# gleb-kov/wordpiece

Hardware: NVIDIA B200
Metric: GB/s text tokenized (higher is better)
Workload: dtype u8

## Files before the change

wordpiece_b200/csrc/wp_encode.cu:

```cuda
#include <cuda_runtime.h>
#include <stddef.h>
#include <stdint.h>

#include "wp_encode.h"
#include "wp_table.h"

#ifdef WP_DEBUG_BOUNDS
#include <cstdio>
#define WP_CHECK(cond)                                                                                              \
  do {                                                                                                              \
    if (!(cond)) {                                                                                                  \
      printf("WP_CHECK failed: %s (wp_encode.cu:%d, block %d, thread %d)\n", #cond, __LINE__, static_cast<int>(blockIdx.x), \
             static_cast<int>(threadIdx.x));                                                                        \
      __trap();                                                                                                     \
    }                                                                                                               \
  } while (0)
#else
#define WP_CHECK(cond) \
  do {                 \
  } while (0)
#endif

namespace wp {

constexpr int TILE = 4096;
constexpr int CHUNK = 32;
constexpr int THREADS = 160;
constexpr int HALO = 256;
constexpr int LOOKAHEAD = 32;
constexpr int LEFT = 16;
constexpr int WINDOW = TILE + HALO;
constexpr int NCHUNK = WINDOW / CHUNK;
constexpr int OWNED_CHUNKS = TILE / CHUNK;
constexpr int RAW_BYTES = LEFT + WINDOW + LOOKAHEAD;
constexpr int WARPS = THREADS / 32;
constexpr int MAX_TILE_SLOW = TILE / 2 + 8;
constexpr int PREFETCH_TILES = 2 * 6 * 148;
constexpr uint32_t FULL = 0xFFFFFFFFu;
constexpr uint32_t POS_MASK = 0x3FFFu;
constexpr uint32_t SLOW_LONG = 0x8000u;

#ifndef WP_K2_BLOCKS
#define WP_K2_BLOCKS 5
#endif
#ifndef WP_K2_THREADS
#define WP_K2_THREADS 256
#endif
#ifndef WP_K1_PER_TURN
#define WP_K1_PER_TURN 2
#endif
#ifndef WP_K3_BLOCKS
#define WP_K3_BLOCKS 4
#endif
#ifndef WP_K1_SEG_CAP
#define WP_K1_SEG_CAP 3072
#endif
constexpr int MATCH_THREADS = WP_K2_THREADS;
constexpr int SCATTER_THREADS = 256;
constexpr int SCATTER_ITEMS = 8;
constexpr int SCATTER_SEGS = SCATTER_THREADS * SCATTER_ITEMS;
constexpr int SCATTER_STAGE = 6144;
#ifndef WP_SCATTER_BIG
#define WP_SCATTER_BIG 8
#endif
constexpr int SCATTER_BIG = WP_SCATTER_BIG;

static_assert(RAW_BYTES % 16 == 0, "raw buffer is loaded in 16-byte units");
static_assert(WORD_KEY_BYTES + 4 <= LOOKAHEAD, "key window reads stay inside the loaded bytes");
static_assert(LONG_SEGMENT_BYTES <= HALO, "a segment that starts in the tile and is not LONG ends inside the window");
static_assert(NCHUNK + 1 <= THREADS, "one thread per chunk in the classification and compaction passes");
static_assert(WINDOW <= static_cast<int>(POS_MASK), "positions must fit the packed list entries");
static_assert(TILE <= 4096, "segment ordinals must fit 12 bits of the tile slow list");
static_assert(NCHUNK < 256, "chunk indices are kept in bytes (hi_list)");

template <int SEG_CAP>
struct __align__(16) TileSmemT {
  uint8_t raw[RAW_BYTES];
  uint16_t seg_s[SEG_CAP];
  uint16_t seg_e[SEG_CAP + HALO + 64];
  uint16_t slow[MAX_TILE_SLOW];
  uint32_t dyn_hits;
  uint32_t n_eligible;
  uint32_t any_single;
  uint32_t m_lead[NCHUNK + 1];
  uint32_t m_space[NCHUNK + 1];
  uint32_t m_punct[NCHUNK + 1];
  uint32_t m_han[NCHUNK + 1];
  uint32_t m_cover[NCHUNK + 1];
  uint32_t m_kept[NCHUNK + 1];
  uint32_t kept_scan[NCHUNK + 2];
  uint8_t spill[NCHUNK + 1];
  uint8_t hi_list[NCHUNK + 8];
  uint32_t n_hi;
  uint32_t tile_ticket;
  uint4 key_mask[WORD_KEY_BYTES + 1];
  uint32_t warp_sums[WARPS];
  uint32_t prev_class;
  uint32_t left_spill;
  uint32_t n_segs;
  uint32_t n_ends;
  uint32_t n_slow;
  uint32_t slow_base;
  uint32_t arena_base;
  unsigned long long seg_base;
};
// ... 277 lines not shown
      sp |= (cls == CLS_SPACE ? 1u : 0u) << j;
      pu |= (cls == CLS_PUNCT ? 1u : 0u) << j;
      ha |= (cls == CLS_HAN ? 1u : 0u) << j;
    }
  } else {
    lead = 0;
    cover = 0;
    spill = 0;
    sp = 0;
    pu = 0;
    for (int j = 0; j < CHUNK; j++) {
      const uint32_t b0 = cb[j];
      if (is_cont_byte(b0)) continue;
      uint32_t cp = 0;
      const uint32_t len = b0 < 0x80u ? (cp = b0, 1u) : utf8_decode(b0, cb[j + 1], cb[j + 2], cb[j + 3], 4u, &cp);
      if (len == 0) continue;
      lead |= 1u << j;
      cover |= ((1u << len) - 1u) << j;
      if (j + static_cast<int>(len) > CHUNK) spill = j + len - CHUNK;
      const uint32_t cls = cp_class(cp);
      sp |= (cls == CLS_SPACE ? 1u : 0u) << j;
      pu |= (cls == CLS_PUNCT ? 1u : 0u) << j;
      ha |= (cls == CLS_HAN ? 1u : 0u) << j;
    }
  }
  const uint32_t in = limit_mask(c, limit);
  sm.m_lead[c] = lead & in;
  sm.m_space[c] = sp & in;
  sm.m_punct[c] = pu & in;
  sm.m_han[c] = ha & in;
  sm.m_cover[c] = cover;
  sm.spill[c] = static_cast<uint8_t>(spill);
}

template <class TileSmem>
__device__ __noinline__ void classify_window(TileSmem &sm, const uint8_t *buf, int limit) {
  const int tid = threadIdx.x;
  const int lane = tid & 31;
  const bool high = tid < NCHUNK && classify_ascii(sm, buf, tid, limit);
  const uint32_t hm = __ballot_sync(FULL, high);
  if (hm) {
    uint32_t at = 0;
    const int leader = __ffs(hm) - 1;
    if (lane == leader) at = smem_add(&sm.n_hi, static_cast<uint32_t>(__popc(hm)));
    at = __shfl_sync(FULL, at, leader);
    WP_CHECK(!high || at + __popc(hm & ((1u << lane) - 1u)) < NCHUNK + 8);
    if (high) sm.hi_list[at + __popc(hm & ((1u << lane) - 1u))] = static_cast<uint8_t>(tid);
  }
  __syncthreads();
  const uint32_t n_hi = sm.n_hi;
  for (uint32_t i = tid; i < n_hi; i += THREADS) classify_multibyte(sm, buf, sm.hi_list[i], limit);
}

template <int NWARPS>
__device__ __forceinline__ uint32_t block_exclusive_scan(uint32_t *warp_sums, uint32_t v, uint32_t *total) {
  const int lane = threadIdx.x & 31, warp = threadIdx.x >> 5;
  uint32_t incl = v;
#pragma unroll
  for (int o = 1; o < 32; o <<= 1) {
    const uint32_t y = __shfl_up_sync(FULL, incl, o);
    if (lane >= o) incl += y;
  }
  __syncthreads();
  if (lane == 31) warp_sums[warp] = incl;
  __syncthreads();
  uint32_t wbase = 0, tot = 0;
#pragma unroll
  for (int wi = 0; wi < NWARPS; wi++) {
    const uint32_t ws = warp_sums[wi];
    if (wi < warp) wbase += ws;
    tot += ws;
  }
  *total = tot;
  return wbase + incl - v;
}

__device__ __noinline__ unsigned long long tile_exclusive_scan(uint32_t *warp_sums, uint32_t v) {
  uint32_t total;
  const uint32_t at = block_exclusive_scan<WARPS>(warp_sums, v, &total);
  return (static_cast<unsigned long long>(total) << 32) | at;
}

__device__ __forceinline__ void lookback_publish(volatile unsigned long long *state, uint32_t index,
                                                 unsigned long long total) {
  state[index] = ((index == 0 ? 2ull : 1ull) << 62) | total;
}

constexpr uint32_t LOOKBACK_SPIN_LIMIT = 1u << 24;

__device__ __forceinline__ unsigned long long lookback_walk(volatile unsigned long long *state, uint32_t index,
                                                            unsigned long long total, int lane,
                                                            unsigned int *stalled = nullptr, unsigned int *void_call = nullptr) {
  constexpr unsigned long long VALUE_MASK = (1ull << 62) - 1;
  unsigned long long base = 0;
  if (index == 0) return 0;
  long long pred = static_cast<long long>(index) - 1 - lane;
  for (;;) {
    unsigned long long sv = 2ull << 62;
    if (pred >= 0) {
      uint32_t spins = 0;
      do {
        sv = state[pred];
        if (++spins > LOOKBACK_SPIN_LIMIT && stalled != nullptr) {
          *stalled = 1u;
          if (void_call != nullptr) *void_call = 1u;
          sv = 2ull << 62;
        }
      } while ((sv >> 62) == 0);
    }
    const uint32_t is_prefix = __ballot_sync(FULL, (sv >> 62) == 2);
    const int stop = is_prefix ? __ffs(is_prefix) - 1 : 31;
    unsigned long long v = lane <= stop ? (sv & VALUE_MASK) : 0ull;
#pragma unroll
    for (int o = 16; o > 0; o >>= 1) v += __shfl_xor_sync(FULL, v, o);
    base += v;
    if (is_prefix) break;
    pred -= 32;
  }
  if (lane == 0) state[index] = (2ull << 62) | (base + total);
  return base;
}

// ... 856 lines not shown
          sm.jump[k][i] = j == LONG_END ? static_cast<uint16_t>(LONG_END) : sm.jump[k - 1][j];
        }
        __syncthreads();
      }
#pragma unroll 1
      for (int k = LONG_LEVELS - 1; k >= 0; k--) {
        for (uint32_t i = tid; i < n; i += LONG_THREADS) {
          const uint32_t r = sm.rank[i];
          if (r == LONG_END) continue;
          const uint32_t j = sm.jump[k][i];
          WP_CHECK(j == LONG_END || (j < n && j > i && r + (1u << k) < LONG_BLOCK));
          if (j != LONG_END) sm.rank[j] = static_cast<uint16_t>(r + (1u << k));
        }
        __syncthreads();
      }
#pragma unroll 1
      for (uint32_t i = tid; i < n; i += LONG_THREADS) {
        const uint32_t r = sm.rank[i];
        if (r == LONG_END) continue;
        const uint32_t dl = sm.delta[i];
        if (dl == 0) {
          sm.failed = 1;
        } else {
          WP_CHECK(static_cast<unsigned long long>(sm.off) + n_out + r < P.arena_capacity && b0 + i - start >= n_out + r);
          out[n_out + r] = sm.id[i];
          if (sm.jump[0][i] == LONG_END) {
            sm.n_round = r + 1;
            sm.cur_next = b0 + i + dl;
          }
        }
      }
      __syncthreads();
      if (tid == 0) {
        sm.n_out = n_out + sm.n_round;
        sm.cur = sm.cur_next;
        if (sm.failed || sm.cur_next >= seg_end) sm.finished = 1;
      }
      __syncthreads();
    }
    if (tid == 0) {
      uint32_t cnt = sm.n_out;
      if (sm.failed) {
        cnt = sm.word_first + 1;
        P.arena[sm.off + sm.word_first] = static_cast<uint32_t>(V.unk_id);
      }
      if (P.call->overflow) cnt = 0;
      *reinterpret_cast<uint4 *>(&P.slow[si]) = make_uint4(cnt, sm.off, 0u, 0u);
      P.seg_result[ent.seg] = SEG_RESULT_SLOW | (min(cnt, SEG_SLOW_COUNT_MAX) << SEG_SLOW_INDEX_BITS) | si;
    }
  }
}


struct ScatterSmem {
  int32_t stage[SCATTER_STAGE];
  uint32_t desc_pos[SCATTER_SEGS];
  uint32_t desc_src[SCATTER_SEGS];
  uint32_t n_desc;
  uint32_t n_big;
  uint16_t big[SCATTER_STAGE / (SCATTER_BIG < 6144 ? SCATTER_BIG : 6144) + 2];
  uint32_t warp_sums[SCATTER_THREADS / 32];
  uint32_t block_index[2];
  unsigned long long base;
};

template <class Params>
__device__ __forceinline__ void scatter_fetch(const Params &P, uint32_t res, uint32_t cnt, int32_t *dst) {
  if (res & SEG_RESULT_SLOW) {
    const uint32_t si = res & SEG_SLOW_INDEX_MASK;
    if (si >= P.slow_capacity) return;
    const uint4 e = *reinterpret_cast<const uint4 *>(&P.slow[si]);
    if (e.x & SLOW_RESULT_INLINE) {
      dst[0] = static_cast<int32_t>(e.y);
      if (cnt > 1) dst[1] = static_cast<int32_t>(e.z);
      if (cnt > 2) dst[2] = static_cast<int32_t>(e.w);
    } else if (static_cast<unsigned long long>(e.y) + cnt <= P.arena_capacity) {
      const int32_t *src = reinterpret_cast<const int32_t *>(P.arena + e.y);
      for (uint32_t t = 0; t < cnt; t++) dst[t] = src[t];
    }
  } else {
    const WordSlot *slot = P.words + (res & SEG_WORD_SLOT_MASK);
    const uint4 e = *reinterpret_cast<const uint4 *>(&slot->meta);
    dst[0] = static_cast<int32_t>(e.y);
    if (cnt > 1) dst[1] = static_cast<int32_t>(e.z);
    if (cnt > 2) dst[2] = static_cast<int32_t>(e.w);
    for (uint32_t t = 3; t < cnt; t++) dst[t] = slot->ids[t];
  }
}

__device__ __forceinline__ void scatter_direct(const EncodeParams &P, unsigned long long first, unsigned long long n_segs,
                                            unsigned long long out0, uint32_t at, uint32_t *big_at, uint32_t *big_si,
                                            uint32_t *n_big) {
  unsigned long long o = out0 + at;
#pragma unroll 1
  for (int j = 0; j < SCATTER_ITEMS; j++) {
    if (first + j >= n_segs) break;
    const uint32_t res = P.seg_result[first + j];
    uint32_t cnt = 1u;
    if (res >= SEG_RESULT_WORD) {
      cnt = (res >> SEG_SLOW_INDEX_BITS) & ((res & SEG_RESULT_SLOW) ? SEG_SLOW_COUNT_MAX : 0xFu);
      if (cnt == SEG_SLOW_COUNT_MAX && (res & SEG_RESULT_SLOW)) {
        const uint32_t si = res & SEG_SLOW_INDEX_MASK;
        cnt = si < P.slow_capacity ? (P.slow[si].off & ~SLOW_RESULT_INLINE) : 0u;
      }
    }
    if (cnt == 0) continue;
    if (res < SEG_RESULT_WORD) {
      if (o < P.capacity) P.ids[o] = static_cast<int32_t>(res) - 1;
    } else if ((res & SEG_RESULT_SLOW) && cnt > SCATTER_BIG && (res & SEG_SLOW_INDEX_MASK) < P.slow_capacity) {
      const uint32_t b = atomicAdd(n_big, 1u);
      big_at[b] = static_cast<uint32_t>(o - out0);
      big_si[b] = res & SEG_SLOW_INDEX_MASK;
    } else if (o + cnt <= P.capacity) {
      scatter_fetch(P, res, cnt, P.ids + o);
    } else {
      int32_t tmp[WORD_MAX_IDS];
      if (cnt <= WORD_MAX_IDS) {
        scatter_fetch(P, res, cnt, tmp);
        for (uint32_t t = 0; t < cnt; t++) {
          if (o + t < P.capacity) P.ids[o + t] = tmp[t];
        }
      } else {
        const uint32_t si = res & SEG_SLOW_INDEX_MASK;
        if (si < P.slow_capacity) {
          const uint4 e = *reinterpret_cast<const uint4 *>(&P.slow[si]);
          if (static_cast<unsigned long long>(e.y) + cnt <= P.arena_capacity) {
            for (uint32_t t = 0; t < cnt; t++) {
              if (o + t < P.capacity) P.ids[o + t] = static_cast<int32_t>(P.arena[e.y + t]);
            }
          }
        }
      }
    }
    o += cnt;
  }
}

constexpr uint32_t MIXED_MAX_BIG = SCATTER_SEGS / 2;

struct ScatterView {
  const uint32_t *seg_result;
  const SlowEntry *slow;
  const uint32_t *arena;
  const WordSlot *words;
  volatile unsigned long long *block_state;
  CallCounters *call;
  int32_t *ids;
  unsigned long long capacity;
  uint32_t slow_capacity, arena_capacity, range_parity;
};

__device__ __noinline__ bool scatter_mixed(const ScatterView P, ScatterSmem &sm, unsigned long long first,
                                           unsigned long long n_segs, uint32_t b, uint32_t n_blocks,
                                           unsigned long long ids_in, uint32_t total, uint32_t at) {
  const int tid = threadIdx.x, lane = tid & 31, warp = tid >> 5;
  auto count_of = [&](uint32_t res) -> uint32_t {
    if (res < SEG_RESULT_WORD) return 1u;
    uint32_t c = (res >> SEG_SLOW_INDEX_BITS) & ((res & SEG_RESULT_SLOW) ? SEG_SLOW_COUNT_MAX : 0xFu);
    if (c == SEG_SLOW_COUNT_MAX && (res & SEG_RESULT_SLOW)) {
      const uint32_t si = res & SEG_SLOW_INDEX_MASK;
      c = si < P.slow_capacity ? (P.slow[si].off & ~SLOW_RESULT_INLINE) : 0u;
    }
    return c;
  };
  auto is_big = [&](uint32_t res, uint32_t c) {
    return (res & SEG_RESULT_SLOW) && res >= SEG_RESULT_WORD && c > SCATTER_BIG && (res & SEG_SLOW_INDEX_MASK) < P.slow_capacity;
  };
  uint32_t my_small = 0, my_big = 0;
#pragma unroll 1
  for (int j = 0; j < SCATTER_ITEMS; j++) {
    if (first + j >= n_segs) break;
    const uint32_t res = P.seg_result[first + j];
    const uint32_t c = count_of(res);
    if (is_big(res, c)) my_big++;
    else my_small += c;
  }
  uint32_t totals;
  const uint32_t ex = block_exclusive_scan<SCATTER_THREADS / 32>(sm.warp_sums, my_small | (my_big << 16), &totals);
  const uint32_t n_small = totals & 0xFFFFu, n_big = totals >> 16;
  if (n_small > SCATTER_STAGE || n_big > MIXED_MAX_BIG || n_big == 0) return false;
  if (warp == 0) {
    const unsigned long long base = lookback_walk(P.block_state, b, total, lane);
    if (lane == 0) {
      sm.base = base;
      if (b == n_blocks - 1) P.call->ids_total[P.range_parity ^ 1u] = ids_in + base + total;
    }
  }
  uint32_t spos = ex & 0xFFFFu, bk = ex >> 16, pos = at;
#pragma unroll 1
  for (int j = 0; j < SCATTER_ITEMS; j++) {
    if (first + j >= n_segs) break;
    const uint32_t res = P.seg_result[first + j];
    const uint32_t c = count_of(res);
    if (c == 0) continue;
    if (res < SEG_RESULT_WORD) {
      sm.stage[spos++] = static_cast<int32_t>(res) - 1;
    } else if (is_big(res, c)) {
      WP_CHECK(bk < MIXED_MAX_BIG);
      sm.desc_pos[bk] = spos;
      sm.desc_pos[MIXED_MAX_BIG + bk] = pos + c - spos;
      sm.desc_src[bk] = res & SEG_SLOW_INDEX_MASK;
      bk++;
    } else {
      WP_CHECK(spos + c <= SCATTER_STAGE);
      scatter_fetch(P, res, c, sm.stage + spos);
      spos += c;
    }
    pos += c;
  }
  __syncthreads();
  const unsigned long long out0 = ids_in + sm.base;
  for (uint32_t i = tid; i < n_small; i += SCATTER_THREADS) {
    uint32_t lo = 0, hi = n_big;
    while (lo < hi) {
      const uint32_t mid = (lo + hi) >> 1;
      if (sm.desc_pos[mid] <= i) lo = mid + 1;
      else hi = mid;
    }
    const uint32_t shift = lo ? sm.desc_pos[MIXED_MAX_BIG + lo - 1] : 0u;
    const unsigned long long o = out0 + i + shift;
    WP_CHECK(i + shift < total);
    if (o < P.capacity) P.ids[o] = sm.stage[i];
  }
  for (uint32_t k = warp; k < n_big; k += SCATTER_THREADS / 32) {
    const uint32_t si = sm.desc_src[k];
    const uint4 e = *reinterpret_cast<const uint4 *>(&P.slow[si]);
    const uint32_t cnt = e.x & ~SLOW_RESULT_INLINE;
    if ((e.x & SLOW_RESULT_INLINE) || static_cast<unsigned long long>(e.y) + cnt > P.arena_capacity) continue;
    const unsigned long long o = out0 + (sm.desc_pos[MIXED_MAX_BIG + k] - cnt + sm.desc_pos[k]);
    WP_CHECK(sm.desc_pos[MIXED_MAX_BIG + k] + sm.desc_pos[k] <= total && sm.desc_pos[MIXED_MAX_BIG + k] + sm.desc_pos[k] >= cnt);
    for (uint32_t t = lane; t < cnt; t += 32) {
      if (o + t < P.capacity) P.ids[o + t] = static_cast<int32_t>(P.arena[e.y + t]);
    }
  }
  return true;
}

__global__ void __launch_bounds__(SCATTER_THREADS, WP_K3_BLOCKS) wp_scatter_kernel(EncodeParams P) {
  __shared__ ScatterSmem sm;
  const int tid = threadIdx.x;
  const int lane = tid & 31;
  const int warp = tid >> 5;
  const unsigned long long n_segs = min(P.counters->n_segs, static_cast<unsigned long long>(P.seg_capacity));
  const uint32_t n_blocks = static_cast<uint32_t>((n_segs + SCATTER_SEGS - 1) / SCATTER_SEGS);
  const unsigned long long ids_in = P.call->ids_total[P.range_parity];
  if (P.call->overflow) return;
  if (n_blocks == 0) {
    if (blockIdx.x == 0 && tid == 0) P.call->ids_total[P.range_parity ^ 1u] = ids_in;
    return;
  }
  if (tid == 0) sm.block_index[0] = atomicAdd(&P.counters->scatter_ticket, 1u);
  for (uint32_t it = 0;; it++) {
    __syncthreads();
    const uint32_t b = sm.block_index[it & 1u];
    if (b >= n_blocks) break;
    if (tid == 0) {
      sm.n_desc = 0;
      sm.n_big = 0;
    }
    const unsigned long long first = static_cast<unsigned long long>(b) * SCATTER_SEGS + tid * SCATTER_ITEMS;
    {
      const unsigned long long pf = (static_cast<unsigned long long>(b) + 2ull * gridDim.x) * SCATTER_SEGS + tid * 32ull;
      if (tid < SCATTER_SEGS / 32 && pf < n_segs) prefetch_l2(P.seg_result + pf);
    }

    uint32_t res[SCATTER_ITEMS], cnt[SCATTER_ITEMS];
    if (first + SCATTER_ITEMS <= n_segs) {
      const uint4 a = *reinterpret_cast<const uint4 *>(P.seg_result + first);
      const uint4 c = *reinterpret_cast<const uint4 *>(P.seg_result + first + 4);
      res[0] = a.x; res[1] = a.y; res[2] = a.z; res[3] = a.w;
      res[4] = c.x; res[5] = c.y; res[6] = c.z; res[7] = c.w;
    } else {
#pragma unroll
      for (int j = 0; j < SCATTER_ITEMS; j++) res[j] = first + j < n_segs ? P.seg_result[first + j] : SEG_RESULT_WORD;
    }
    uint32_t mine = 0, n_other = 0;
#pragma unroll
    for (int j = 0; j < SCATTER_ITEMS; j++) {
      uint32_t c = 1u;
      if (res[j] >= SEG_RESULT_WORD) {
        c = (res[j] >> SEG_SLOW_INDEX_BITS) & ((res[j] & SEG_RESULT_SLOW) ? SEG_SLOW_COUNT_MAX : 0xFu);
        if (c == SEG_SLOW_COUNT_MAX && (res[j] & SEG_RESULT_SLOW)) {
          const uint32_t si = res[j] & SEG_SLOW_INDEX_MASK;
          c = si < P.slow_capacity ? (P.slow[si].off & ~SLOW_RESULT_INLINE) : 0u;
        }
        n_other += c != 0u;
      }
      cnt[j] = c;
      mine += c;
    }
    uint32_t total;
    uint32_t at = block_exclusive_scan<SCATTER_THREADS / 32>(sm.warp_sums, mine, &total);

    if (tid == 0) lookback_publish(P.block_state, b, total);

    if (total <= SCATTER_STAGE) {
      uint32_t d = n_other;
#pragma unroll
      for (int o = 1; o < 32; o <<= 1) {
        const uint32_t y = __shfl_up_sync(FULL, d, o);
        if (lane >= o) d += y;
      }
      uint32_t wbase = 0;
      if (lane == 31 && d) wbase = smem_add(&sm.n_desc, d);
      d = d - n_other + __shfl_sync(FULL, wbase, 31);
#pragma unroll
      for (int j = 0; j < SCATTER_ITEMS; j++) {
        WP_CHECK(at + cnt[j] <= total && total <= SCATTER_STAGE);
        if (res[j] < SEG_RESULT_WORD) {
          sm.stage[at] = static_cast<int32_t>(res[j]) - 1;
        } else if (cnt[j] != 0) {
          WP_CHECK(d < SCATTER_SEGS);
          sm.desc_pos[d] = (at << 16) | cnt[j];
          sm.desc_src[d] = res[j];
          d++;
        }
        at += cnt[j];
      }
      __syncthreads();
      const uint32_t n_desc = sm.n_desc;
      for (uint32_t i = tid; i < n_desc; i += SCATTER_THREADS) {
        const uint32_t dp = sm.desc_pos[i], src = sm.desc_src[i];
        if ((src & SEG_RESULT_SLOW) && (dp & 0xFFFFu) > SCATTER_BIG) {
          const uint32_t slot = atomicAdd(&sm.n_big, 1u);
          WP_CHECK(slot < SCATTER_STAGE / SCATTER_BIG + 2);
          sm.big[slot] = static_cast<uint16_t>(i);
        } else {
          scatter_fetch(P, src, dp & 0xFFFFu, sm.stage + (dp >> 16));
        }
      }
      if (warp == 0) {
        const unsigned long long base = lookback_walk(P.block_state, b, total, lane);
        if (lane == 0) {
          sm.base = base;
          if (b == n_blocks - 1) P.call->ids_total[P.range_parity ^ 1u] = ids_in + base + total;
        }
      }
      __syncthreads();
      if (sm.n_big) {
        for (uint32_t bi = warp; bi < sm.n_big; bi += SCATTER_THREADS / 32) {
          const uint32_t dp = sm.desc_pos[sm.big[bi]], si = sm.desc_src[sm.big[bi]] & SEG_SLOW_INDEX_MASK;
          if (si >= P.slow_capacity) continue;
          const uint4 e = *reinterpret_cast<const uint4 *>(&P.slow[si]);
          const uint32_t cnt = dp & 0xFFFFu;
          if ((e.x & SLOW_RESULT_INLINE) || static_cast<unsigned long long>(e.y) + cnt > P.arena_capacity) continue;
          for (uint32_t t = lane; t < cnt; t += 32) sm.stage[(dp >> 16) + t] = static_cast<int32_t>(P.arena[e.y + t]);
        }
        __syncthreads();
      }
      if (tid == 0) sm.block_index[(it + 1u) & 1u] = atomicAdd(&P.counters->scatter_ticket, 1u);
      const unsigned long long out0 = ids_in + sm.base;
      if (out0 + total <= P.capacity) {
        int32_t *dst = P.ids + out0;
        const uint32_t head = min(total, static_cast<uint32_t>((4u - ((reinterpret_cast<uintptr_t>(dst) >> 2) & 3u)) & 3u));
        const uint32_t n_vec = (total - head) >> 2;
        if (tid < head) dst[tid] = sm.stage[tid];
        for (uint32_t q = tid; q < n_vec; q += SCATTER_THREADS) {
          const uint32_t i = head + 4u * q;
          *reinterpret_cast<int4 *>(dst + i) = make_int4(sm.stage[i], sm.stage[i + 1], sm.stage[i + 2], sm.stage[i + 3]);
        }
        const uint32_t done = head + 4u * n_vec;
        if (tid < total - done) dst[done + tid] = sm.stage[done + tid];
      } else {
        for (uint32_t i = tid; i < total; i += SCATTER_THREADS) {
          if (out0 + i < P.capacity) P.ids[out0 + i] = sm.stage[i];
        }
      }
    } else {
      const ScatterView view{P.seg_result, P.slow, P.arena, P.words, P.block_state, P.call, P.ids,
                             static_cast<unsigned long long>(P.capacity), P.slow_capacity, P.arena_capacity, P.range_parity};
      if (scatter_mixed(view, sm, first, n_segs, b, n_blocks, ids_in, total, at)) {
        if (tid == 0) sm.block_index[(it + 1u) & 1u] = atomicAdd(&P.counters->scatter_ticket, 1u);
        continue;
      }
      if (warp == 0) {
        const unsigned long long base = lookback_walk(P.block_state, b, total, lane);
        if (lane == 0) {
          sm.base = base;
          if (b == n_blocks - 1) P.call->ids_total[P.range_parity ^ 1u] = ids_in + base + total;
        }
      }
      __syncthreads();
      const unsigned long long out0 = ids_in + sm.base;
      scatter_direct(P, first, n_segs, out0, at, sm.desc_pos, sm.desc_src, &sm.n_big);
      __syncthreads();
      for (uint32_t bi = warp; bi < sm.n_big; bi += SCATTER_THREADS / 32) {
        const uint32_t si = sm.desc_src[bi];
        const unsigned long long o = out0 + sm.desc_pos[bi];
        const uint4 e = *reinterpret_cast<const uint4 *>(&P.slow[si]);
        const uint32_t cnt = e.x & ~SLOW_RESULT_INLINE;
        if ((e.x & SLOW_RESULT_INLINE) || static_cast<unsigned long long>(e.y) + cnt > P.arena_capacity) continue;
        for (uint32_t t = lane; t < cnt; t += 32) {
          if (o + t < P.capacity) P.ids[o + t] = static_cast<int32_t>(P.arena[e.y + t]);
        }
      }
      if (tid == 0) sm.block_index[(it + 1u) & 1u] = atomicAdd(&P.counters->scatter_ticket, 1u);
    }
  }
}

__device__ __forceinline__ uint32_t seg_id_count(const EncodeParams &P, uint32_t res) {
  if (res < SEG_RESULT_WORD) return 1u;
  uint32_t c = (res >> SEG_SLOW_INDEX_BITS) & ((res & SEG_RESULT_SLOW) ? SEG_SLOW_COUNT_MAX : 0xFu);
  if (c == SEG_SLOW_COUNT_MAX && (res & SEG_RESULT_SLOW)) {
    const uint32_t si = res & SEG_SLOW_INDEX_MASK;
    c = si < P.slow_capacity ? (P.slow[si].off & ~SLOW_RESULT_INLINE) : 0u;
  }
  return c;
}

constexpr int OFFSET_THREADS = 128;

__global__ void __launch_bounds__(OFFSET_THREADS) wp_text_offsets_kernel(EncodeParams P, uint32_t i0, uint32_t i1) {
  const int lane = threadIdx.x & 31;
  const uint32_t i = i0 + blockIdx.x * (OFFSET_THREADS / 32) + (threadIdx.x >> 5);
  if (i >= i1 || P.call->overflow) return;
  const unsigned long long n_segs = min(P.counters->n_segs, static_cast<unsigned long long>(P.seg_capacity));
  const unsigned long long s = min(static_cast<unsigned long long>(P.bound_seg[i]), n_segs);
  const uint32_t blk = static_cast<uint32_t>(s / SCATTER_SEGS);
  const unsigned long long first = static_cast<unsigned long long>(blk) * SCATTER_SEGS;
  unsigned long long sum = 0;
  for (unsigned long long k = first + lane; k < s; k += 32) sum += seg_id_count(P, P.seg_result[k]);
#pragma unroll
  for (int o = 16; o > 0; o >>= 1) sum += __shfl_xor_sync(FULL, sum, o);
  if (lane == 0) {
    const unsigned long long before = blk ? (P.block_state[blk - 1] & ((1ull << 62) - 1)) : 0ull;
    P.id_offsets[i] = P.call->ids_total[P.range_parity] + before + sum;
  }
}

cudaError_t launch_text_offsets(const EncodeParams &P, uint32_t i0, uint32_t i1, cudaStream_t stream, uint64_t *launches) {
  if (i1 <= i0) return cudaSuccess;
  const uint32_t per = OFFSET_THREADS / 32;
  wp_text_offsets_kernel<<<(i1 - i0 + per - 1) / per, OFFSET_THREADS, 0, stream>>>(P, i0, i1);
  if (launches) *launches += 1;
  return cudaGetLastError();
}


constexpr int FORMAT_THREADS = 256;
constexpr int FORMAT_ITEMS = 8;
constexpr int FORMAT_IDS = FORMAT_THREADS * FORMAT_ITEMS;
constexpr int FORMAT_MAX_CHARS = 12;

__device__ __forceinline__ uint32_t decimal_chars(int32_t v) {
  const uint32_t a = v < 0 ? 0u - static_cast<uint32_t>(v) : static_cast<uint32_t>(v);
  uint32_t n = 2u + (v < 0 ? 1u : 0u);
  n += a >= 10u;
  n += a >= 100u;
  n += a >= 1000u;
  n += a >= 10000u;
  n += a >= 100000u;
  n += a >= 1000000u;
  n += a >= 10000000u;
  n += a >= 100000000u;
  n += a >= 1000000000u;
  return n;
}

__global__ void __launch_bounds__(FORMAT_THREADS) wp_format_total_kernel(const int32_t *__restrict__ ids,
                                                                         unsigned long long n,
                                                                         unsigned long long *total) {
// ... 99 lines not shown
  uint4 *dst = reinterpret_cast<uint4 *>(work + idx);
  dst[0] = key;
  dst[2] = src[2];
  dst[3] = src[3];
  dst[1] = lo;
}

cudaError_t launch_seed_words(const WordSlot *image, uint32_t image_slots, WordSlot *work, uint32_t work_slots_log2,
                              cudaStream_t stream, uint64_t *launches) {
  cudaError_t e = cudaMemsetAsync(work, 0, (size_t(1) << work_slots_log2) * sizeof(WordSlot), stream);
  if (e != cudaSuccess) return e;
  wp_seed_words_kernel<<<(image_slots + 255) / 256, 256, 0, stream>>>(image, image_slots, work,
                                                                      (1u << work_slots_log2) - 1u, 32 - work_slots_log2);
  if (launches) *launches += 1;
  return cudaGetLastError();
}

__global__ void wp_publish_count_kernel(const CallCounters *call, uint32_t parity, unsigned long long *out) {
  *out = call->overflow ? ~0ull : call->ids_total[parity];
}

cudaError_t launch_publish_count(const CallCounters *call, uint32_t parity, unsigned long long *d_out, cudaStream_t stream,
                                 uint64_t *launches) {
  wp_publish_count_kernel<<<1, 1, 0, stream>>>(call, parity, d_out);
  if (launches) *launches += 1;
  return cudaGetLastError();
}


uint32_t encode_tile_bytes() { return TILE; }
uint32_t scatter_block_segments() { return SCATTER_SEGS; }
size_t kernel_geometry(uint32_t *out, size_t cap) {
  const uint32_t g[] = {TILE, LONG_SEGMENT_BYTES, WP_K1_SEG_CAP, SCATTER_SEGS, SCATTER_STAGE, SCATTER_BIG, MIXED_MAX_BIG,
                        LONG_BLOCK, WORD_KEY_BYTES, WORD_MAX_IDS, SEG_SLOW_COUNT_MAX,
                        3u };
  const size_t n = sizeof(g) / sizeof(g[0]);
  for (size_t i = 0; i < n && i < cap; i++) out[i] = g[i];
  return n;
}

cudaError_t launch_encode_range(const EncodeParams &P, int sm_count, cudaStream_t stream, uint64_t *launches,
                                cudaEvent_t *timing) {
  static bool configured[64] = {false};
  int dev = 0;
  cudaError_t e = cudaGetDevice(&dev);
  if (e != cudaSuccess) return e;
  if (dev < 0 || dev >= 64 || !configured[dev]) {
    e = cudaFuncSetAttribute(wp_split_kernel<WP_K1_SEG_CAP>, cudaFuncAttributeMaxDynamicSharedMemorySize,
                             static_cast<int>(sizeof(TileSmemT<WP_K1_SEG_CAP>)));
    if (e != cudaSuccess) return e;
    e = cudaFuncSetAttribute(wp_split_kernel<TILE>, cudaFuncAttributeMaxDynamicSharedMemorySize,
                             static_cast<int>(sizeof(TileSmemT<TILE>)));
    if (e != cudaSuccess) return e;
    if (dev >= 0 && dev < 64) configured[dev] = true;
  }
  if (sm_count <= 0) sm_count = 148;
  cudaLaunchAttribute attr[1];
  auto window = [&](const void *base, size_t bytes, float ratio) -> unsigned {
    if (bytes == 0) return 0;
    attr[0].id = cudaLaunchAttributeAccessPolicyWindow;
    attr[0].val.accessPolicyWindow.base_ptr = const_cast<void *>(base);
    attr[0].val.accessPolicyWindow.num_bytes = bytes;
    attr[0].val.accessPolicyWindow.hitRatio = ratio;
    attr[0].val.accessPolicyWindow.hitProp = cudaAccessPropertyPersisting;
    attr[0].val.accessPolicyWindow.missProp = cudaAccessPropertyStreaming;
    return 1;
  };
  cudaLaunchConfig_t cfg{};
  cfg.stream = stream;
  cfg.attrs = attr;

  if (timing) cudaEventRecord(timing[0], stream);
  cfg.gridDim = dim3(P.n_tiles);
  cfg.blockDim = dim3(THREADS);
  cfg.numAttrs = window(P.words, P.persist_words_bytes, P.persist_words_ratio);
  if (P.dense_tiles) {
    cfg.dynamicSmemBytes = sizeof(TileSmemT<TILE>);
    e = cudaLaunchKernelEx(&cfg, wp_split_kernel<TILE>, P);
  } else {
    cfg.dynamicSmemBytes = sizeof(TileSmemT<WP_K1_SEG_CAP>);
    e = cudaLaunchKernelEx(&cfg, wp_split_kernel<WP_K1_SEG_CAP>, P);
  }
  if (e != cudaSuccess) return e;
  if (launches) *launches += 1;
  if (timing) cudaEventRecord(timing[1], stream);

  cfg.gridDim = dim3(min(static_cast<unsigned>(sm_count * WP_K2_BLOCKS), P.n_tiles * 4u));
  cfg.blockDim = dim3(MATCH_THREADS);
  cfg.dynamicSmemBytes = 0;
  cfg.numAttrs = window(P.vocab.edges, P.persist_edges_bytes, P.persist_edges_ratio);
  e = cudaLaunchKernelEx(&cfg, wp_match_kernel, P);
  if (e != cudaSuccess) return e;

  cfg.gridDim = dim3(min(static_cast<unsigned>(sm_count * 8), P.n_tiles * 2u + 2u));
  cfg.blockDim = dim3(LONG_THREADS);
  e = cudaLaunchKernelEx(&cfg, wp_long_kernel, P);
  if (e != cudaSuccess) return e;
  if (launches) *launches += 2;
  if (timing) cudaEventRecord(timing[2], stream);

  cfg.gridDim = dim3(min(static_cast<unsigned>(sm_count * WP_K3_BLOCKS), P.n_tiles * 2u));
  cfg.blockDim = dim3(SCATTER_THREADS);
  cfg.dynamicSmemBytes = 0;
  cfg.numAttrs = window(P.words, P.persist_words_bytes, P.persist_words_ratio);
  e = cudaLaunchKernelEx(&cfg, wp_scatter_kernel, P);
  if (e != cudaSuccess) return e;
// ... 7 lines not shown
```

Measured before the change: 152.5.

## Overlap scatter id fetches with lookback walk and parallelize tail fetches

The scatter kernel now computes descriptor indices and tail-id keys with one 64-bit block scan instead of a shared atomic counter. It splits each block so warp 0 does the decoupled lookback walk while the other warps fetch word and slow-segment ids into the stage buffer in parallel, with a flat binary-search over tail ids. Shared state shrinks (16-bit segment indices, no big list), K3 blocks per SM go from 4 to 5, and a shared-memory carveout is set for the higher occupancy. The risks are more complex index packing with 12-bit fields and the loss of one warp for fetching.

```diff
diff --git a/wordpiece_b200/csrc/wp_encode.cu b/wordpiece_b200/csrc/wp_encode.cu
--- a/wordpiece_b200/csrc/wp_encode.cu
+++ b/wordpiece_b200/csrc/wp_encode.cu
@@ -50,7 +50,7 @@
 #define WP_K1_PER_TURN 2
 #endif
 #ifndef WP_K3_BLOCKS
-#define WP_K3_BLOCKS 4
+#define WP_K3_BLOCKS 5
 #endif
 #ifndef WP_K1_SEG_CAP
 #define WP_K1_SEG_CAP 3072
@@ -434,22 +434,22 @@
   for (uint32_t i = tid; i < n_hi; i += THREADS) classify_multibyte(sm, buf, sm.hi_list[i], limit);
 }
 
-template <int NWARPS>
-__device__ __forceinline__ uint32_t block_exclusive_scan(uint32_t *warp_sums, uint32_t v, uint32_t *total) {
+template <int NWARPS, class T>
+__device__ __forceinline__ T block_exclusive_scan(T *warp_sums, T v, T *total) {
   const int lane = threadIdx.x & 31, warp = threadIdx.x >> 5;
-  uint32_t incl = v;
+  T incl = v;
 #pragma unroll
   for (int o = 1; o < 32; o <<= 1) {
-    const uint32_t y = __shfl_up_sync(FULL, incl, o);
+    const T y = __shfl_up_sync(FULL, incl, o);
     if (lane >= o) incl += y;
   }
   __syncthreads();
   if (lane == 31) warp_sums[warp] = incl;
   __syncthreads();
-  uint32_t wbase = 0, tot = 0;
+  T wbase = 0, tot = 0;
 #pragma unroll
   for (int wi = 0; wi < NWARPS; wi++) {
-    const uint32_t ws = warp_sums[wi];
+    const T ws = warp_sums[wi];
     if (wi < warp) wbase += ws;
     tot += ws;
   }
@@ -1412,84 +1412,167 @@
 }
 
 
+template <class Params>
+__device__ __forceinline__ uint32_t seg_id_count(const Params &P, uint32_t res) {
+  if (res < SEG_RESULT_WORD) return 1u;
+  uint32_t c = (res >> SEG_SLOW_INDEX_BITS) & ((res & SEG_RESULT_SLOW) ? SEG_SLOW_COUNT_MAX : 0xFu);
+  if (c == SEG_SLOW_COUNT_MAX && (res & SEG_RESULT_SLOW)) {
+    const uint32_t si = res & SEG_SLOW_INDEX_MASK;
+    c = si < P.slow_capacity ? (P.slow[si].off & ~SLOW_RESULT_INLINE) : 0u;
+  }
+  return c;
+}
+
+constexpr uint32_t SRC_NONE = 0;
+constexpr uint32_t SRC_WORD = 1;
+constexpr uint32_t SRC_INLINE = 2;
+constexpr uint32_t SRC_ARENA = 3;
+constexpr uint32_t DESC_POS_MASK = 0xFFFFu;
+static_assert(SCATTER_STAGE < (1 << 16) && SCATTER_SEGS <= (1 << 16), "stage positions and keys fit 16 bits of desc_pos");
+
 struct ScatterSmem {
   int32_t stage[SCATTER_STAGE];
   uint32_t desc_pos[SCATTER_SEGS];
-  uint32_t desc_src[SCATTER_SEGS];
-  uint32_t n_desc;
+  uint16_t desc_seg[SCATTER_SEGS];
   uint32_t n_big;
-  uint16_t big[SCATTER_STAGE / (SCATTER_BIG < 6144 ? SCATTER_BIG : 6144) + 2];
-  uint32_t warp_sums[SCATTER_THREADS / 32];
+  unsigned long long warp_sums[SCATTER_THREADS / 32];
   uint32_t block_index[2];
   unsigned long long base;
 };
 
 template <class Params>
-__device__ __forceinline__ void scatter_fetch(const Params &P, uint32_t res, uint32_t cnt, int32_t *dst) {
-  if (res & SEG_RESULT_SLOW) {
-    const uint32_t si = res & SEG_SLOW_INDEX_MASK;
-    if (si >= P.slow_capacity) return;
-    const uint4 e = *reinterpret_cast<const uint4 *>(&P.slow[si]);
-    if (e.x & SLOW_RESULT_INLINE) {
-      dst[0] = static_cast<int32_t>(e.y);
-      if (cnt > 1) dst[1] = static_cast<int32_t>(e.z);
-      if (cnt > 2) dst[2] = static_cast<int32_t>(e.w);
-    } else if (static_cast<unsigned long long>(e.y) + cnt <= P.arena_capacity) {
-      const int32_t *src = reinterpret_cast<const int32_t *>(P.arena + e.y);
-      for (uint32_t t = 0; t < cnt; t++) dst[t] = src[t];
-    }
+__device__ __forceinline__ uint32_t resolve_slow(const Params &P, uint32_t si, uint32_t cnt, uint32_t *where, uint4 *e_out) {
+  if (si >= P.slow_capacity) return SRC_NONE;
+  const uint4 e = *reinterpret_cast<const uint4 *>(&P.slow[si]);
+  *e_out = e;
+  if (e.x & SLOW_RESULT_INLINE) {
+    *where = si;
+    return SRC_INLINE;
+  }
+  if (static_cast<unsigned long long>(e.y) + cnt > P.arena_capacity) return SRC_NONE;
+  *where = e.y;
+  return SRC_ARENA;
+}
+
+template <class Params>
+__device__ __forceinline__ bool source_id(const Params &P, uint32_t kind, uint32_t where, uint32_t t, int32_t *v) {
+  if (kind == SRC_WORD) {
+    *v = P.words[where].ids[t];
+  } else if (kind == SRC_ARENA) {
+    *v = static_cast<int32_t>(P.arena[where + t]);
+  } else if (kind == SRC_INLINE && t < 3) {
+    *v = reinterpret_cast<const int32_t *>(&P.slow[where])[1 + t];
   } else {
-    const WordSlot *slot = P.words + (res & SEG_WORD_SLOT_MASK);
-    const uint4 e = *reinterpret_cast<const uint4 *>(&slot->meta);
-    dst[0] = static_cast<int32_t>(e.y);
-    if (cnt > 1) dst[1] = static_cast<int32_t>(e.z);
-    if (cnt > 2) dst[2] = static_cast<int32_t>(e.w);
-    for (uint32_t t = 3; t < cnt; t++) dst[t] = slot->ids[t];
+    return false;
+  }
+  return true;
+}
+
+__device__ __forceinline__ uint32_t tail_ids(uint32_t res, uint32_t c) {
+  return c > 3u ? ((res & SEG_RESULT_SLOW) ? c : c - 3u) : 0u;
+}
+
+__device__ __forceinline__ void list_segment(ScatterSmem &sm, uint32_t d, uint32_t key, uint32_t spos, uint32_t seg) {
+  WP_CHECK(d < SCATTER_SEGS && spos < SCATTER_STAGE && key <= SCATTER_STAGE);
+  sm.desc_pos[d] = (key << 16) | spos;
+  sm.desc_seg[d] = static_cast<uint16_t>(seg);
+}
+
+template <class Params>
+__device__ __forceinline__ void fetch_beside_walk(const Params &P, ScatterSmem &sm, uint32_t n_desc, uint32_t n_tail,
+                                                  uint32_t b, uint32_t n_blocks, unsigned long long ids_in,
+                                                  uint32_t total) {
+  constexpr uint32_t FETCH_THREADS = SCATTER_THREADS - 32;
+  const uint32_t tid = threadIdx.x;
+  if (tid < 32) {
+    const unsigned long long base = lookback_walk(P.block_state, b, total, static_cast<int>(tid));
+    if (tid == 0) {
+      sm.base = base;
+      if (b == n_blocks - 1) P.call->ids_total[P.range_parity ^ 1u] = ids_in + base + total;
+    }
+    return;
+  }
+  const uint32_t *seg_result = P.seg_result + static_cast<unsigned long long>(b) * SCATTER_SEGS;
+  auto tail_of = [&](uint32_t k, uint32_t dp) {
+    return (k + 1 < n_desc ? sm.desc_pos[k + 1] >> 16 : n_tail) - (dp >> 16);
+  };
+  for (uint32_t k = tid - 32; k < n_desc; k += FETCH_THREADS) {
+    const uint32_t dp = sm.desc_pos[k], res = seg_result[sm.desc_seg[k]], spos = dp & DESC_POS_MASK;
+    const uint32_t tail = tail_of(k, dp);
+    uint32_t cnt, e1 = 0, e2 = 0, e3 = 0;
+    bool have = true;
+    if (!(res & SEG_RESULT_SLOW)) {
+      cnt = (res >> SEG_SLOW_INDEX_BITS) & 0xFu;
+      const uint4 e = *reinterpret_cast<const uint4 *>(&P.words[res & SEG_WORD_SLOT_MASK].meta);
+      e1 = e.y, e2 = e.z, e3 = e.w;
+    } else {
+      cnt = tail ? tail : (res >> SEG_SLOW_INDEX_BITS) & SEG_SLOW_COUNT_MAX;
+      uint32_t where = 0;
+      uint4 e;
+      const uint32_t kind = resolve_slow(P, res & SEG_SLOW_INDEX_MASK, cnt, &where, &e);
+      if (kind == SRC_INLINE) {
+        e1 = e.y, e2 = e.z, e3 = e.w;
+      } else if (kind == SRC_ARENA && !tail) {
+        e1 = P.arena[where];
+        if (cnt > 1) e2 = P.arena[where + 1];
+        if (cnt > 2) e3 = P.arena[where + 2];
+      } else {
+        have = false;
+      }
+    }
+    if (have) {
+      WP_CHECK(spos + min(cnt, 3u) <= SCATTER_STAGE);
+      sm.stage[spos] = static_cast<int32_t>(e1);
+      if (cnt > 1) sm.stage[spos + 1] = static_cast<int32_t>(e2);
+      if (cnt > 2) sm.stage[spos + 2] = static_cast<int32_t>(e3);
+    }
+  }
+  for (uint32_t i = tid - 32; i < n_tail; i += FETCH_THREADS) {
+    uint32_t lo = 0, hi = n_desc;
+    while (hi - lo > 1) {
+      const uint32_t mid = (lo + hi) >> 1;
+      if ((sm.desc_pos[mid] >> 16) <= i) lo = mid;
+      else hi = mid;
+    }
+    const uint32_t dp = sm.desc_pos[lo], res = seg_result[sm.desc_seg[lo]];
+    uint32_t t = i - (dp >> 16), kind = SRC_WORD, where = res & SEG_WORD_SLOT_MASK;
+    if (res & SEG_RESULT_SLOW) {
+      uint4 e;
+      kind = resolve_slow(P, res & SEG_SLOW_INDEX_MASK, tail_of(lo, dp), &where, &e);
+    } else {
+      t += 3u;
+    }
+    int32_t v;
+    if (source_id(P, kind, where, t, &v)) {
+      WP_CHECK((dp & DESC_POS_MASK) + t < SCATTER_STAGE);
+      sm.stage[(dp & DESC_POS_MASK) + t] = v;
+    }
   }
 }
 
 __device__ __forceinline__ void scatter_direct(const EncodeParams &P, unsigned long long first, unsigned long long n_segs,
-                                            unsigned long long out0, uint32_t at, uint32_t *big_at, uint32_t *big_si,
+                                            unsigned long long out0, uint32_t at, uint32_t *big_at, uint16_t *big_seg,
                                             uint32_t *n_big) {
   unsigned long long o = out0 + at;
 #pragma unroll 1
   for (int j = 0; j < SCATTER_ITEMS; j++) {
     if (first + j >= n_segs) break;
     const uint32_t res = P.seg_result[first + j];
-    uint32_t cnt = 1u;
-    if (res >= SEG_RESULT_WORD) {
-      cnt = (res >> SEG_SLOW_INDEX_BITS) & ((res & SEG_RESULT_SLOW) ? SEG_SLOW_COUNT_MAX : 0xFu);
-      if (cnt == SEG_SLOW_COUNT_MAX && (res & SEG_RESULT_SLOW)) {
-        const uint32_t si = res & SEG_SLOW_INDEX_MASK;
-        cnt = si < P.slow_capacity ? (P.slow[si].off & ~SLOW_RESULT_INLINE) : 0u;
-      }
-    }
+    const uint32_t cnt = seg_id_count(P, res);
     if (cnt == 0) continue;
     if (res < SEG_RESULT_WORD) {
       if (o < P.capacity) P.ids[o] = static_cast<int32_t>(res) - 1;
     } else if ((res & SEG_RESULT_SLOW) && cnt > SCATTER_BIG && (res & SEG_SLOW_INDEX_MASK) < P.slow_capacity) {
       const uint32_t b = atomicAdd(n_big, 1u);
       big_at[b] = static_cast<uint32_t>(o - out0);
-      big_si[b] = res & SEG_SLOW_INDEX_MASK;
-    } else if (o + cnt <= P.capacity) {
-      scatter_fetch(P, res, cnt, P.ids + o);
+      big_seg[b] = static_cast<uint16_t>(threadIdx.x * SCATTER_ITEMS + j);
     } else {
-      int32_t tmp[WORD_MAX_IDS];
-      if (cnt <= WORD_MAX_IDS) {
-        scatter_fetch(P, res, cnt, tmp);
-        for (uint32_t t = 0; t < cnt; t++) {
-          if (o + t < P.capacity) P.ids[o + t] = tmp[t];
-        }
-      } else {
-        const uint32_t si = res & SEG_SLOW_INDEX_MASK;
-        if (si < P.slow_capacity) {
-          const uint4 e = *reinterpret_cast<const uint4 *>(&P.slow[si]);
-          if (static_cast<unsigned long long>(e.y) + cnt <= P.arena_capacity) {
-            for (uint32_t t = 0; t < cnt; t++) {
-              if (o + t < P.capacity) P.ids[o + t] = static_cast<int32_t>(P.arena[e.y + t]);
-            }
-          }
-        }
+      uint32_t where = res & SEG_WORD_SLOT_MASK;
+      uint4 e;
+      const uint32_t kind = (res & SEG_RESULT_SLOW) ? resolve_slow(P, res & SEG_SLOW_INDEX_MASK, cnt, &where, &e) : SRC_WORD;
+      for (uint32_t t = 0; t < cnt; t++) {
+        int32_t v;
+        if (o + t < P.capacity && source_id(P, kind, where, t, &v)) P.ids[o + t] = v;
       }
     }
     o += cnt;
@@ -1512,83 +1595,99 @@
 
 __device__ __noinline__ bool scatter_mixed(const ScatterView P, ScatterSmem &sm, unsigned long long first,
                                            unsigned long long n_segs, uint32_t b, uint32_t n_blocks,
-                                           unsigned long long ids_in, uint32_t total, uint32_t at) {
+                                           unsigned long long ids_in, uint32_t total) {
   const int tid = threadIdx.x, lane = tid & 31, warp = tid >> 5;
-  auto count_of = [&](uint32_t res) -> uint32_t {
-    if (res < SEG_RESULT_WORD) return 1u;
-    uint32_t c = (res >> SEG_SLOW_INDEX_BITS) & ((res & SEG_RESULT_SLOW) ? SEG_SLOW_COUNT_MAX : 0xFu);
-    if (c == SEG_SLOW_COUNT_MAX && (res & SEG_RESULT_SLOW)) {
-      const uint32_t si = res & SEG_SLOW_INDEX_MASK;
-      c = si < P.slow_capacity ? (P.slow[si].off & ~SLOW_RESULT_INLINE) : 0u;
-    }
-    return c;
-  };
   auto is_big = [&](uint32_t res, uint32_t c) {
     return (res & SEG_RESULT_SLOW) && res >= SEG_RESULT_WORD && c > SCATTER_BIG && (res & SEG_SLOW_INDEX_MASK) < P.slow_capacity;
   };
-  uint32_t my_small = 0, my_big = 0;
+  uint32_t my_small = 0, my_big = 0, my_list = 0, my_tail = 0;
 #pragma unroll 1
   for (int j = 0; j < SCATTER_ITEMS; j++) {
     if (first + j >= n_segs) break;
     const uint32_t res = P.seg_result[first + j];
-    const uint32_t c = count_of(res);
-    if (is_big(res, c)) my_big++;
-    else my_small += c;
-  }
-  uint32_t totals;
-  const uint32_t ex = block_exclusive_scan<SCATTER_THREADS / 32>(sm.warp_sums, my_small | (my_big << 16), &totals);
-  const uint32_t n_small = totals & 0xFFFFu, n_big = totals >> 16;
+    const uint32_t c = seg_id_count(P, res);
+    if (is_big(res, c)) {
+      my_big++;
+    } else {
+      my_small += c;
+      if (res >= SEG_RESULT_WORD && c != 0) {
+        my_list++;
+        my_tail += tail_ids(res, c);
+      }
+    }
+  }
+  unsigned long long totals;
+  const unsigned long long ex = block_exclusive_scan<SCATTER_THREADS / 32>(
+      sm.warp_sums, my_small | (my_big << 16) | (static_cast<unsigned long long>(my_list) << 32) |
+                        (static_cast<unsigned long long>(my_tail) << 44), &totals);
+  const uint32_t n_small = totals & 0xFFFFu, n_big = (totals >> 16) & 0xFFFu;
+  const uint32_t n_list = (totals >> 32) & 0xFFFu, n_tail = static_cast<uint32_t>(totals >> 44);
   if (n_small > SCATTER_STAGE || n_big > MIXED_MAX_BIG || n_big == 0) return false;
-  if (warp == 0) {
-    const unsigned long long base = lookback_walk(P.block_state, b, total, lane);
-    if (lane == 0) {
-      sm.base = base;
-      if (b == n_blocks - 1) P.call->ids_total[P.range_parity ^ 1u] = ids_in + base + total;
-    }
-  }
-  uint32_t spos = ex & 0xFFFFu, bk = ex >> 16, pos = at;
+  uint32_t spos = ex & 0xFFFFu, bk = (ex >> 16) & 0xFFFu;
+  uint32_t d = (ex >> 32) & 0xFFFu, key = static_cast<uint32_t>(ex >> 44);
 #pragma unroll 1
   for (int j = 0; j < SCATTER_ITEMS; j++) {
     if (first + j >= n_segs) break;
     const uint32_t res = P.seg_result[first + j];
-    const uint32_t c = count_of(res);
+    const uint32_t c = seg_id_count(P, res);
     if (c == 0) continue;
+    const uint32_t seg = static_cast<uint32_t>(tid * SCATTER_ITEMS + j);
     if (res < SEG_RESULT_WORD) {
       sm.stage[spos++] = static_cast<int32_t>(res) - 1;
     } else if (is_big(res, c)) {
-      WP_CHECK(bk < MIXED_MAX_BIG);
-      sm.desc_pos[bk] = spos;
-      sm.desc_pos[MIXED_MAX_BIG + bk] = pos + c - spos;
-      sm.desc_src[bk] = res & SEG_SLOW_INDEX_MASK;
-      bk++;
+      WP_CHECK(bk < MIXED_MAX_BIG && n_list + bk < SCATTER_SEGS);
+      sm.desc_pos[SCATTER_SEGS - 1 - bk++] = (spos << 16) | seg;
     } else {
       WP_CHECK(spos + c <= SCATTER_STAGE);
-      scatter_fetch(P, res, c, sm.stage + spos);
+      list_segment(sm, d++, key, spos, seg);
+      key += tail_ids(res, c);
       spos += c;
     }
-    pos += c;
+  }
+  __syncthreads();
+  fetch_beside_walk(P, sm, n_list, n_tail, b, n_blocks, ids_in, total);
+  const uint32_t *seg_result = P.seg_result + static_cast<unsigned long long>(b) * SCATTER_SEGS;
+  constexpr uint32_t BIG_PER_THREAD = MIXED_MAX_BIG / SCATTER_THREADS;
+  static_assert(MIXED_MAX_BIG % SCATTER_THREADS == 0 && 2 * MIXED_MAX_BIG <= SCATTER_SEGS, "long-segment lists");
+  uint32_t c_big[BIG_PER_THREAD], my_ids = 0;
+#pragma unroll
+  for (uint32_t q = 0; q < BIG_PER_THREAD; q++) {
+    const uint32_t k = tid * BIG_PER_THREAD + q;
+    c_big[q] = k < n_big ? seg_id_count(P, seg_result[sm.desc_pos[SCATTER_SEGS - 1 - k] & 0xFFFFu]) : 0u;
+    my_ids += c_big[q];
+  }
+  unsigned long long big_total;
+  uint32_t shift = static_cast<uint32_t>(block_exclusive_scan<SCATTER_THREADS / 32>(
+      sm.warp_sums, static_cast<unsigned long long>(my_ids), &big_total));
+#pragma unroll
+  for (uint32_t q = 0; q < BIG_PER_THREAD; q++) {
+    const uint32_t k = tid * BIG_PER_THREAD + q;
+    shift += c_big[q];
+    if (k < n_big) sm.desc_pos[k] = shift;
   }
   __syncthreads();
   const unsigned long long out0 = ids_in + sm.base;
+  auto big_key = [&](uint32_t k) { return sm.desc_pos[SCATTER_SEGS - 1 - k]; };
   for (uint32_t i = tid; i < n_small; i += SCATTER_THREADS) {
     uint32_t lo = 0, hi = n_big;
     while (lo < hi) {
       const uint32_t mid = (lo + hi) >> 1;
-      if (sm.desc_pos[mid] <= i) lo = mid + 1;
+      if ((big_key(mid) >> 16) <= i) lo = mid + 1;
       else hi = mid;
     }
-    const uint32_t shift = lo ? sm.desc_pos[MIXED_MAX_BIG + lo - 1] : 0u;
-    const unsigned long long o = out0 + i + shift;
-    WP_CHECK(i + shift < total);
+    const uint32_t sh = lo ? sm.desc_pos[lo - 1] : 0u;
+    const unsigned long long o = out0 + i + sh;
+    WP_CHECK(i + sh < total);
     if (o < P.capacity) P.ids[o] = sm.stage[i];
   }
   for (uint32_t k = warp; k < n_big; k += SCATTER_THREADS / 32) {
-    const uint32_t si = sm.desc_src[k];
+    const uint32_t si = seg_result[big_key(k) & 0xFFFFu] & SEG_SLOW_INDEX_MASK;
     const uint4 e = *reinterpret_cast<const uint4 *>(&P.slow[si]);
     const uint32_t cnt = e.x & ~SLOW_RESULT_INLINE;
     if ((e.x & SLOW_RESULT_INLINE) || static_cast<unsigned long long>(e.y) + cnt > P.arena_capacity) continue;
-    const unsigned long long o = out0 + (sm.desc_pos[MIXED_MAX_BIG + k] - cnt + sm.desc_pos[k]);
-    WP_CHECK(sm.desc_pos[MIXED_MAX_BIG + k] + sm.desc_pos[k] <= total && sm.desc_pos[MIXED_MAX_BIG + k] + sm.desc_pos[k] >= cnt);
+    const uint32_t end = sm.desc_pos[k] + (big_key(k) >> 16);
+    const unsigned long long o = out0 + (end - cnt);
+    WP_CHECK(end <= total && end >= cnt);
     for (uint32_t t = lane; t < cnt; t += 32) {
       if (o + t < P.capacity) P.ids[o + t] = static_cast<int32_t>(P.arena[e.y + t]);
     }
@@ -1614,17 +1713,14 @@
     __syncthreads();
     const uint32_t b = sm.block_index[it & 1u];
     if (b >= n_blocks) break;
-    if (tid == 0) {
-      sm.n_desc = 0;
-      sm.n_big = 0;
-    }
+    if (tid == 0) sm.n_big = 0;
     const unsigned long long first = static_cast<unsigned long long>(b) * SCATTER_SEGS + tid * SCATTER_ITEMS;
     {
       const unsigned long long pf = (static_cast<unsigned long long>(b) + 2ull * gridDim.x) * SCATTER_SEGS + tid * 32ull;
       if (tid < SCATTER_SEGS / 32 && pf < n_segs) prefetch_l2(P.seg_result + pf);
     }
 
-    uint32_t res[SCATTER_ITEMS], cnt[SCATTER_ITEMS];
+    uint32_t res[SCATTER_ITEMS];
     if (first + SCATTER_ITEMS <= n_segs) {
       const uint4 a = *reinterpret_cast<const uint4 *>(P.seg_result + first);
       const uint4 c = *reinterpret_cast<const uint4 *>(P.seg_result + first + 4);
@@ -1634,80 +1730,43 @@
 #pragma unroll
       for (int j = 0; j < SCATTER_ITEMS; j++) res[j] = first + j < n_segs ? P.seg_result[first + j] : SEG_RESULT_WORD;
     }
-    uint32_t mine = 0, n_other = 0;
+    uint32_t mine = 0, n_list = 0, n_tail = 0;
 #pragma unroll
     for (int j = 0; j < SCATTER_ITEMS; j++) {
-      uint32_t c = 1u;
+      const uint32_t c = seg_id_count(P, res[j]);
       if (res[j] >= SEG_RESULT_WORD) {
-        c = (res[j] >> SEG_SLOW_INDEX_BITS) & ((res[j] & SEG_RESULT_SLOW) ? SEG_SLOW_COUNT_MAX : 0xFu);
-        if (c == SEG_SLOW_COUNT_MAX && (res[j] & SEG_RESULT_SLOW)) {
-          const uint32_t si = res[j] & SEG_SLOW_INDEX_MASK;
-          c = si < P.slow_capacity ? (P.slow[si].off & ~SLOW_RESULT_INLINE) : 0u;
-        }
-        n_other += c != 0u;
-      }
-      cnt[j] = c;
+        n_list += c != 0u;
+        n_tail += tail_ids(res[j], c);
+      }
       mine += c;
     }
-    uint32_t total;
-    uint32_t at = block_exclusive_scan<SCATTER_THREADS / 32>(sm.warp_sums, mine, &total);
+    unsigned long long totals;
+    const unsigned long long ex = block_exclusive_scan<SCATTER_THREADS / 32>(
+        sm.warp_sums, mine | (static_cast<unsigned long long>(n_list) << 32) | (static_cast<unsigned long long>(n_tail) << 44),
+        &totals);
+    const uint32_t total = static_cast<uint32_t>(totals);
+    uint32_t at = static_cast<uint32_t>(ex);
 
     if (tid == 0) lookback_publish(P.block_state, b, total);
 
     if (total <= SCATTER_STAGE) {
-      uint32_t d = n_other;
-#pragma unroll
-      for (int o = 1; o < 32; o <<= 1) {
-        const uint32_t y = __shfl_up_sync(FULL, d, o);
-        if (lane >= o) d += y;
-      }
-      uint32_t wbase = 0;
-      if (lane == 31 && d) wbase = smem_add(&sm.n_desc, d);
-      d = d - n_other + __shfl_sync(FULL, wbase, 31);
+      uint32_t d = (ex >> 32) & 0xFFFu, key = static_cast<uint32_t>(ex >> 44);
 #pragma unroll
       for (int j = 0; j < SCATTER_ITEMS; j++) {
-        WP_CHECK(at + cnt[j] <= total && total <= SCATTER_STAGE);
+        const uint32_t c = seg_id_count(P, res[j]);
+        WP_CHECK(at + c <= total && total <= SCATTER_STAGE);
         if (res[j] < SEG_RESULT_WORD) {
           sm.stage[at] = static_cast<int32_t>(res[j]) - 1;
-        } else if (cnt[j] != 0) {
-          WP_CHECK(d < SCATTER_SEGS);
-          sm.desc_pos[d] = (at << 16) | cnt[j];
-          sm.desc_src[d] = res[j];
-          d++;
-        }
-        at += cnt[j];
+        } else if (c != 0) {
+          list_segment(sm, d++, key, at, static_cast<uint32_t>(tid * SCATTER_ITEMS + j));
+          key += tail_ids(res[j], c);
+        }
+        at += c;
       }
       __syncthreads();
-      const uint32_t n_desc = sm.n_desc;
-      for (uint32_t i = tid; i < n_desc; i += SCATTER_THREADS) {
-        const uint32_t dp = sm.desc_pos[i], src = sm.desc_src[i];
-        if ((src & SEG_RESULT_SLOW) && (dp & 0xFFFFu) > SCATTER_BIG) {
-          const uint32_t slot = atomicAdd(&sm.n_big, 1u);
-          WP_CHECK(slot < SCATTER_STAGE / SCATTER_BIG + 2);
-          sm.big[slot] = static_cast<uint16_t>(i);
-        } else {
-          scatter_fetch(P, src, dp & 0xFFFFu, sm.stage + (dp >> 16));
-        }
-      }
-      if (warp == 0) {
-        const unsigned long long base = lookback_walk(P.block_state, b, total, lane);
-        if (lane == 0) {
-          sm.base = base;
-          if (b == n_blocks - 1) P.call->ids_total[P.range_parity ^ 1u] = ids_in + base + total;
-        }
-      }
+      fetch_beside_walk(P, sm, static_cast<uint32_t>(totals >> 32) & 0xFFFu, static_cast<uint32_t>(totals >> 44), b,
+                        n_blocks, ids_in, total);
       __syncthreads();
-      if (sm.n_big) {
-        for (uint32_t bi = warp; bi < sm.n_big; bi += SCATTER_THREADS / 32) {
-          const uint32_t dp = sm.desc_pos[sm.big[bi]], si = sm.desc_src[sm.big[bi]] & SEG_SLOW_INDEX_MASK;
-          if (si >= P.slow_capacity) continue;
-          const uint4 e = *reinterpret_cast<const uint4 *>(&P.slow[si]);
-          const uint32_t cnt = dp & 0xFFFFu;
-          if ((e.x & SLOW_RESULT_INLINE) || static_cast<unsigned long long>(e.y) + cnt > P.arena_capacity) continue;
-          for (uint32_t t = lane; t < cnt; t += 32) sm.stage[(dp >> 16) + t] = static_cast<int32_t>(P.arena[e.y + t]);
-        }
-        __syncthreads();
-      }
       if (tid == 0) sm.block_index[(it + 1u) & 1u] = atomicAdd(&P.counters->scatter_ticket, 1u);
       const unsigned long long out0 = ids_in + sm.base;
       if (out0 + total <= P.capacity) {
@@ -1729,7 +1788,7 @@
     } else {
       const ScatterView view{P.seg_result, P.slow, P.arena, P.words, P.block_state, P.call, P.ids,
                              static_cast<unsigned long long>(P.capacity), P.slow_capacity, P.arena_capacity, P.range_parity};
-      if (scatter_mixed(view, sm, first, n_segs, b, n_blocks, ids_in, total, at)) {
+      if (scatter_mixed(view, sm, first, n_segs, b, n_blocks, ids_in, total)) {
         if (tid == 0) sm.block_index[(it + 1u) & 1u] = atomicAdd(&P.counters->scatter_ticket, 1u);
         continue;
       }
@@ -1742,10 +1801,10 @@
       }
       __syncthreads();
       const unsigned long long out0 = ids_in + sm.base;
-      scatter_direct(P, first, n_segs, out0, at, sm.desc_pos, sm.desc_src, &sm.n_big);
+      scatter_direct(P, first, n_segs, out0, at, sm.desc_pos, sm.desc_seg, &sm.n_big);
       __syncthreads();
       for (uint32_t bi = warp; bi < sm.n_big; bi += SCATTER_THREADS / 32) {
-        const uint32_t si = sm.desc_src[bi];
+        const uint32_t si = P.seg_result[static_cast<unsigned long long>(b) * SCATTER_SEGS + sm.desc_seg[bi]] & SEG_SLOW_INDEX_MASK;
         const unsigned long long o = out0 + sm.desc_pos[bi];
         const uint4 e = *reinterpret_cast<const uint4 *>(&P.slow[si]);
         const uint32_t cnt = e.x & ~SLOW_RESULT_INLINE;
@@ -1759,15 +1818,6 @@
   }
 }
 
-__device__ __forceinline__ uint32_t seg_id_count(const EncodeParams &P, uint32_t res) {
-  if (res < SEG_RESULT_WORD) return 1u;
-  uint32_t c = (res >> SEG_SLOW_INDEX_BITS) & ((res & SEG_RESULT_SLOW) ? SEG_SLOW_COUNT_MAX : 0xFu);
-  if (c == SEG_SLOW_COUNT_MAX && (res & SEG_RESULT_SLOW)) {
-    const uint32_t si = res & SEG_SLOW_INDEX_MASK;
-    c = si < P.slow_capacity ? (P.slow[si].off & ~SLOW_RESULT_INLINE) : 0u;
-  }
-  return c;
-}
 
 constexpr int OFFSET_THREADS = 128;
 
@@ -1973,6 +2023,9 @@
     e = cudaFuncSetAttribute(wp_split_kernel<TILE>, cudaFuncAttributeMaxDynamicSharedMemorySize,
                              static_cast<int>(sizeof(TileSmemT<TILE>)));
     if (e != cudaSuccess) return e;
+    e = cudaFuncSetAttribute(wp_scatter_kernel, cudaFuncAttributePreferredSharedMemoryCarveout,
+                             static_cast<int>((WP_K3_BLOCKS * (sizeof(ScatterSmem) + 1024) * 100 + 233471) / 233472));
+    if (e != cudaSuccess) return e;
     if (dev >= 0 && dev < 64) configured[dev] = true;
   }
   if (sm_count <= 0) sm_count = 148;
```

Result: no change. 153.0 (median of 6 runs) (+0.4%).
